# duylebkHCM/doc2tex

Hardware: AMD Instinct MI355X
Metric: formulas/s (greedy decode, 128x512 crops) (higher is better)
Workload: dtype bf16x3

## Files before the change

doc2tex_amd/csrc/decode.hip:

```cpp
#include <cstdlib>

#include "kernels.h"

namespace d2t {

using f32x4 = __attribute__((ext_vector_type(4))) float;
#ifndef D2T_DECODE_PRIO
#define D2T_DECODE_PRIO 3
#endif

__device__ __forceinline__ void decode_wave_priority() { __builtin_amdgcn_s_setprio(D2T_DECODE_PRIO); }

struct TraceScope {
  unsigned long long* t;
  __device__ __forceinline__ explicit TraceScope(unsigned long long* tr) : t(tr) {
    if (t && threadIdx.x == 0) atomicMin(t, (unsigned long long)__builtin_amdgcn_s_memrealtime());
  }
  __device__ __forceinline__ ~TraceScope() {
    if (t) {
      __syncthreads();
      if (threadIdx.x == 0) atomicMax(t + 1, (unsigned long long)__builtin_amdgcn_s_memrealtime());
    }
  }
};

__device__ __forceinline__ float act_fn(float v, int act) {
  if (act == ACT_RELU) return fmaxf(v, 0.f);
  if (act == ACT_GELU) return 0.5f * v * (1.f + erff(v * 0.70710678118654752440f));
  return v;
}

template <int NW, int NCH, int MT>
__global__ __launch_bounds__(NW * 64) void skinny_splitk_kernel(const SkinnyP p) {
  if (p.stop_at && *p.stop_at && *p.cur_step >= *p.stop_at) return;
  decode_wave_priority();
  TraceScope trace_(p.trace);
  constexpr int KS = NCH * 16;
  constexpr int ROWS = 16 * MT;
  __shared__ float part[NW][ROWS][17];
  __shared__ float stat[NW][ROWS];
  __shared__ float s_mean[ROWS], s_rstd[ROWS];
  const int tid = threadIdx.x, wave = tid >> 6, lane = tid & 63;
  const int r = lane & 15, q = lane >> 4;
  const int mbase = blockIdx.y * ROWS;
  const int n = blockIdx.x * 16 + r;
  const bool nok = n < p.N;
  const int k0 = wave * KS + q * 4;

  float4 a[MT][NCH], b[NCH];
#pragma unroll
  for (int i = 0; i < MT; ++i) {
    const int m = mbase + i * 16 + r;
    const bool mok = m < p.M;
    const float* src = p.x + (size_t)(mok ? m : 0) * p.ldx + k0;
#pragma unroll
    for (int c = 0; c < NCH; ++c) {
      a[i][c] = *reinterpret_cast<const float4*>(src + c * 16);
      if (!mok) a[i][c] = make_float4(0.f, 0.f, 0.f, 0.f);
    }
  }
  {
    const float* src = p.w + (size_t)(nok ? n : 0) * (p.wld ? p.wld : p.K) + k0;
#pragma unroll
    for (int c = 0; c < NCH; ++c) {
      b[c] = *reinterpret_cast<const float4*>(src + c * 16);
      if (!nok) b[c] = make_float4(0.f, 0.f, 0.f, 0.f);
    }
  }

  if (p.ln_g) {
    const float invK = 1.f / (float)p.K;
#pragma unroll
    for (int i = 0; i < MT; ++i) {
      float s = 0.f;
#pragma unroll
      for (int c = 0; c < NCH; ++c) s += (a[i][c].x + a[i][c].y) + (a[i][c].z + a[i][c].w);
      s += __shfl_xor(s, 16, 64);
      s += __shfl_xor(s, 32, 64);
      if (q == 0) stat[wave][i * 16 + r] = s;
    }
    __syncthreads();
    if (tid < ROWS) {
      float t = 0.f;
#pragma unroll
      for (int w = 0; w < NW; ++w) t += stat[w][tid];
      s_mean[tid] = t * invK;
    }
    __syncthreads();
#pragma unroll
    for (int i = 0; i < MT; ++i) {
      const float mu = s_mean[i * 16 + r];
      float s = 0.f;
#pragma unroll
      for (int c = 0; c < NCH; ++c) {
        a[i][c].x -= mu; a[i][c].y -= mu; a[i][c].z -= mu; a[i][c].w -= mu;
        s += (a[i][c].x * a[i][c].x + a[i][c].y * a[i][c].y) + (a[i][c].z * a[i][c].z + a[i][c].w * a[i][c].w);
      }
      s += __shfl_xor(s, 16, 64);
      s += __shfl_xor(s, 32, 64);
      if (q == 0) stat[wave][i * 16 + r] = s;
    }
    __syncthreads();
    if (tid < ROWS) {
      float t = 0.f;
#pragma unroll
      for (int w = 0; w < NW; ++w) t += stat[w][tid];
      s_rstd[tid] = 1.f / sqrtf(t * invK + p.ln_eps);
    }
    __syncthreads();
#pragma unroll
    for (int c = 0; c < NCH; ++c) {
      const float4 g4 = *reinterpret_cast<const float4*>(p.ln_g + k0 + c * 16);
      const float4 b4 = *reinterpret_cast<const float4*>(p.ln_b + k0 + c * 16);
#pragma unroll
      for (int i = 0; i < MT; ++i) {
        const float rs = s_rstd[i * 16 + r];
        a[i][c].x = a[i][c].x * rs * g4.x + b4.x;
        a[i][c].y = a[i][c].y * rs * g4.y + b4.y;
        a[i][c].z = a[i][c].z * rs * g4.z + b4.z;
        a[i][c].w = a[i][c].w * rs * g4.w + b4.w;
      }
    }
  }

  f32x4 acc[MT];
#pragma unroll
  for (int i = 0; i < MT; ++i) acc[i] = f32x4{0.f, 0.f, 0.f, 0.f};
#pragma unroll
  for (int c = 0; c < NCH; ++c) {
#pragma unroll
    for (int i = 0; i < MT; ++i) {
      acc[i] = __builtin_amdgcn_mfma_f32_16x16x4f32(a[i][c].x, b[c].x, acc[i], 0, 0, 0);
      acc[i] = __builtin_amdgcn_mfma_f32_16x16x4f32(a[i][c].y, b[c].y, acc[i], 0, 0, 0);
      acc[i] = __builtin_amdgcn_mfma_f32_16x16x4f32(a[i][c].z, b[c].z, acc[i], 0, 0, 0);
      acc[i] = __builtin_amdgcn_mfma_f32_16x16x4f32(a[i][c].w, b[c].w, acc[i], 0, 0, 0);
    }
  }
#pragma unroll
  for (int i = 0; i < MT; ++i)
#pragma unroll
    for (int reg = 0; reg < 4; ++reg) part[wave][i * 16 + q * 4 + reg][r] = acc[i][reg];
  __syncthreads();

  float* y = p.y;
  if (p.step_ptr) y += (long long)(*p.step_ptr) * p.out_step_stride;
  for (int idx = tid; idx < ROWS * 16; idx += NW * 64) {
    const int row = idx >> 4, col = idx & 15;
    const int m = mbase + row, nn = blockIdx.x * 16 + col;
    if (m >= p.M || nn >= p.N) continue;
    float v = 0.f;
#pragma unroll
    for (int w = 0; w < NW; ++w) v += part[w][row][col];
    v += p.bias ? p.bias[nn] : 0.f;
    if (p.res) v += p.res[(size_t)m * p.ldres + nn];
    y[(size_t)m * p.ldy + nn] = act_fn(v, p.act);
    if (p.ln_out && nn < p.K) {
      const float xv = p.x[(size_t)m * p.ldx + nn];
      p.ln_out[(size_t)m * p.K + nn] = (xv - s_mean[row]) * s_rstd[row] * p.ln_g[nn] + p.ln_b[nn];
    }
  }
}

__global__ __launch_bounds__(256) void skinny_generic_kernel(const SkinnyP p) {
  const int wave = threadIdx.x >> 6, lane = threadIdx.x & 63;
  const int r = lane & 15, q = lane >> 4;
  const int m = blockIdx.y * 64 + wave * 16 + r;
  const int n = blockIdx.x * 16 + r;
  const bool mok = m < p.M, nok = n < p.N;
  const float* xa = p.x + (size_t)(mok ? m : 0) * p.ldx + q * 4;
  const float* wb = p.w + (size_t)(nok ? n : 0) * p.K + q * 4;
  f32x4 acc = {0.f, 0.f, 0.f, 0.f};
  const int KC = p.K >> 4;
  for (int c = 0; c < KC; ++c) {
    float4 a = *reinterpret_cast<const float4*>(xa + c * 16);
    float4 b = *reinterpret_cast<const float4*>(wb + c * 16);
    if (!mok) a = make_float4(0.f, 0.f, 0.f, 0.f);
    if (!nok) b = make_float4(0.f, 0.f, 0.f, 0.f);
    acc = __builtin_amdgcn_mfma_f32_16x16x4f32(a.x, b.x, acc, 0, 0, 0);
    acc = __builtin_amdgcn_mfma_f32_16x16x4f32(a.y, b.y, acc, 0, 0, 0);
    acc = __builtin_amdgcn_mfma_f32_16x16x4f32(a.z, b.z, acc, 0, 0, 0);
    acc = __builtin_amdgcn_mfma_f32_16x16x4f32(a.w, b.w, acc, 0, 0, 0);
  }
  const int nn = blockIdx.x * 16 + r;
  if (nn >= p.N) return;
  float* y = p.y;
  if (p.step_ptr) y += (long long)(*p.step_ptr) * p.out_step_stride;
  const float bias = p.bias ? p.bias[nn] : 0.f;
#pragma unroll
  for (int reg = 0; reg < 4; ++reg) {
    const int mm = blockIdx.y * 64 + wave * 16 + q * 4 + reg;
    if (mm >= p.M) continue;
    float v = acc[reg] + bias;
    if (p.res) v += p.res[(size_t)mm * p.ldres + nn];
    y[(size_t)mm * p.ldy + nn] = act_fn(v, p.act);
  }
}

static int decode_small() {
  static const int v = D2T_PROBE_ENV("D2T_DECODE_SMALL");
  return v;
}

hipError_t launch_skinny(const SkinnyP& p, hipStream_t s) {
  if (p.M <= 0 || p.N <= 0) return hipSuccess;
  if (p.K % 16 != 0 || p.ldx % 4 != 0) return hipErrorInvalidValue;
  if (p.ln_out && (!p.ln_g || p.N < p.K)) return hipErrorInvalidValue;
  const int mt = p.N <= 512 ? 1 : 2;
  const dim3 grid((p.N + 15) / 16, (p.M + 16 * mt - 1) / (16 * mt));
#define D2T_SK(NW, NCH)                                                                                  \
  do {                                                                                                   \
    if (mt == 1) hipLaunchKernelGGL((skinny_splitk_kernel<NW, NCH, 1>), grid, dim3(NW * 64), 0, s, p);   \
    else hipLaunchKernelGGL((skinny_splitk_kernel<NW, NCH, 2>), grid, dim3(NW * 64), 0, s, p);           \
  } while (0)
  if (p.K == 256) D2T_SK(4, 4);
  else if (p.K == 512) D2T_SK(8, 4);
  else if (p.K == 1024 && decode_small() && !p.ln_g && !p.step_ptr) {
    SkinnyP a = p, b = p;
    a.K = 512; a.ldx = p.ldx; a.w = p.w; a.wld = p.K;
    b.K = 512; b.x = p.x + 512; b.w = p.w + 512; b.wld = p.K; b.bias = nullptr; b.res = p.y; b.ldres = p.ldy;
    a.act = ACT_NONE;
    if (p.act != ACT_NONE) return hipErrorInvalidValue;
    hipLaunchKernelGGL((skinny_splitk_kernel<4, 8, 1>), dim3((p.N + 15) / 16, (p.M + 15) / 16), dim3(256), 0, s, a);
    hipLaunchKernelGGL((skinny_splitk_kernel<4, 8, 1>), dim3((p.N + 15) / 16, (p.M + 15) / 16), dim3(256), 0, s, b);
  }
  else if (p.K == 1024) D2T_SK(8, 8);
  else {
    if (p.ln_g) return hipErrorInvalidValue;
    hipLaunchKernelGGL(skinny_generic_kernel, dim3((p.N + 15) / 16, (p.M + 63) / 64), dim3(256), 0, s, p);
  }
#undef D2T_SK
  return hipGetLastError();
}

template <int HD>
__global__ __launch_bounds__(256) void decode_attention_kernel(const DecAttnP p) {
  constexpr int LPK = HD / 4;
  constexpr int KPI = 64 / LPK;
  constexpr int MAXIT = 512 / (KPI * 4);
  __shared__ float w_m[4], w_s[4];
  __shared__ __attribute__((aligned(16))) float w_acc[4][HD];
  const int tid = threadIdx.x, wave = tid >> 6, lane = tid & 63;
  const int kig = lane / LPK, ch = lane % LPK;
  const int b = blockIdx.x / p.heads, head = blockIdx.x % p.heads;
  int L = p.L, t = -1;
  if (p.step_ptr) { t = *p.step_ptr; L = t + 1; }
  float* Kc = p.k + (size_t)b * p.kv_batch_stride + (size_t)head * p.Lmax * HD;
  float* Vc = p.v + (size_t)b * p.kv_batch_stride + (size_t)head * p.Lmax * HD;
  const float* curk = p.cur_k ? p.cur_k + (size_t)b * p.cur_stride + head * HD : nullptr;
  const float* curv = p.cur_v ? p.cur_v + (size_t)b * p.cur_stride + head * HD : nullptr;
  if (curk && t >= 0 && tid < HD) {
    Kc[(size_t)t * HD + tid] = curk[tid];
    Vc[(size_t)t * HD + tid] = curv[tid];
  }
  const float4 q4 = *reinterpret_cast<const float4*>(p.q + (size_t)b * p.q_stride + head * HD + ch * 4);
  const float scale = HD == 32 ? 0.17677669529663687f : 0.125f;
  const int nit = (L + KPI * 4 - 1) / (KPI * 4);

  float sc[MAXIT];
  float mloc = -INFINITY;
#pragma unroll
  for (int it = 0; it < MAXIT; ++it) {
    sc[it] = -INFINITY;
    if (it < nit) {
      const int j = (it * 4 + wave) * KPI + kig;
      float d = 0.f;
      if (j < L) {
        const float* kr = (curk && j == t) ? curk : Kc + (size_t)j * HD;
        const float4 k4 = *reinterpret_cast<const float4*>(kr + ch * 4);
        d = (q4.x * k4.x + q4.y * k4.y) + (q4.z * k4.z + q4.w * k4.w);
      }
#pragma unroll
      for (int o = 1; o < LPK; o <<= 1) d += __shfl_xor(d, o, 64);
      if (j < L) {
        sc[it] = d * scale;
        mloc = fmaxf(mloc, sc[it]);
      }
    }
  }
#pragma unroll
  for (int o = LPK; o < 64; o <<= 1) mloc = fmaxf(mloc, __shfl_xor(mloc, o, 64));
  float4 acc = make_float4(0.f, 0.f, 0.f, 0.f);
  float ssum = 0.f;
#pragma unroll
  for (int it = 0; it < MAXIT; ++it) {
    if (it < nit) {
      const int j = (it * 4 + wave) * KPI + kig;
      if (j < L) {
        const float pj = expf(sc[it] - mloc);
        const float* vr = (curv && j == t) ? curv : Vc + (size_t)j * HD;
        const float4 v4 = *reinterpret_cast<const float4*>(vr + ch * 4);
        ssum += pj;
        acc.x = fmaf(pj, v4.x, acc.x); acc.y = fmaf(pj, v4.y, acc.y);
        acc.z = fmaf(pj, v4.z, acc.z); acc.w = fmaf(pj, v4.w, acc.w);
      }
    }
  }
#pragma unroll
  for (int o = LPK; o < 64; o <<= 1) {
    ssum += __shfl_xor(ssum, o, 64);
    acc.x += __shfl_xor(acc.x, o, 64); acc.y += __shfl_xor(acc.y, o, 64);
    acc.z += __shfl_xor(acc.z, o, 64); acc.w += __shfl_xor(acc.w, o, 64);
  }
  if (kig == 0) *reinterpret_cast<float4*>(&w_acc[wave][ch * 4]) = acc;
  if (lane == 0) { w_m[wave] = mloc; w_s[wave] = ssum; }
  __syncthreads();
  if (tid < HD) {
    const float m = fmaxf(fmaxf(w_m[0], w_m[1]), fmaxf(w_m[2], w_m[3]));
    float tot = 0.f, o = 0.f;
#pragma unroll
    for (int w = 0; w < 4; ++w) {
      const float f = w_s[w] > 0.f ? expf(w_m[w] - m) : 0.f;
      tot += w_s[w] * f;
      o += w_acc[w][tid] * f;
    }
    p.y[(size_t)b * p.y_stride + head * HD + tid] = o / tot;
  }
}

hipError_t launch_decode_attention(const DecAttnP& p, hipStream_t s) {
  const int Lcap = p.step_ptr ? p.Lmax : p.L;
  if (Lcap > 512 || Lcap < 1) return hipErrorInvalidValue;
  const dim3 grid(p.B * p.heads);
  if (p.hd == 32) hipLaunchKernelGGL(decode_attention_kernel<32>, grid, dim3(256), 0, s, p);
  else if (p.hd == 64) hipLaunchKernelGGL(decode_attention_kernel<64>, grid, dim3(256), 0, s, p);
  else return hipErrorInvalidValue;
  return hipGetLastError();
}

__global__ void embed_kernel(const float* __restrict__ emb, const float* __restrict__ pe,
                             const int64_t* __restrict__ start, const int64_t* __restrict__ tokens, int tok_stride,
                             const int* __restrict__ step_ptr, float* __restrict__ x, int d, float sqrt_d) {
  const int b = blockIdx.x, t = *step_ptr;
  const int64_t tok = t == 0 ? start[b] : tokens[(size_t)b * tok_stride + t - 1];
  for (int c = threadIdx.x; c < d; c += blockDim.x)
    x[(size_t)b * d + c] = emb[(size_t)tok * d + c] * sqrt_d + pe[(size_t)t * d + c];
}

hipError_t launch_embed(const float* emb, const float* pe, const int64_t* start, const int64_t* tokens,
                        int tok_stride, const int* step_ptr, float* x, int B, int d, hipStream_t s) {
  hipLaunchKernelGGL(embed_kernel, dim3(B), dim3(256), 0, s, emb, pe, start, tokens, tok_stride, step_ptr, x, d,
                     sqrtf((float)d));
  return hipGetLastError();
}

__global__ __launch_bounds__(64) void argmax_embed_kernel(const ArgmaxP p) {
  const int t = *p.step_ptr;
  if (p.stop_at && *p.stop_at && t >= *p.stop_at) return;
  decode_wave_priority();
  TraceScope trace_(p.trace);
  const int b = blockIdx.x, lane = threadIdx.x;
  const float* row = p.logits + (size_t)b * p.row_stride + (size_t)t * p.step_stride;
  float best = -INFINITY;
  int bi = 0x7fffffff;
  for (int i = lane; i < p.V; i += 64) {
    const float v = row[i];
    if (v > best || (v == best && i < bi)) { best = v; bi = i; }
  }
#pragma unroll
  for (int o = 32; o > 0; o >>= 1) {
    const float ov = __shfl_xor(best, o, 64);
    const int oi = __shfl_xor(bi, o, 64);
    if (ov > best || (ov == best && oi < bi)) { best = ov; bi = oi; }
  }
  if (bi >= p.V) bi = 0;
  if (p.x) {
    const float sqrt_d = sqrtf((float)p.d);
    const float* e = p.emb + (size_t)bi * p.d;
    const float* pe = p.pe + (size_t)(t + 1) * p.d;
    for (int c = lane; c < p.d; c += 64) p.x[(size_t)b * p.d + c] = e[c] * sqrt_d + pe[c];
  }
  if (lane == 0) {
    p.tokens[(size_t)b * p.tok_stride + t] = bi;
    if (bi == p.end_token && !p.ended[b]) {
      p.ended[b] = 1;
      const int c = atomicAdd(p.end_count, 1) + 1;
      if (c == p.B) *p.steps_done = t + 1;
      if (p.n_batches > 0) {
        const int k = p.row_batch ? p.row_batch[b] : b / p.rows_per_batch;
        const int rows_k = p.batch_rows ? p.batch_rows[k] : p.rows_per_batch;
        const int nb = p.n_batches_ptr ? *p.n_batches_ptr : p.n_batches;
        if (atomicAdd(p.batch_end_count + k, 1) + 1 == rows_k) {
          p.batch_steps_done[k] = t + 1;
          if (atomicAdd(p.batches_done, 1) + 1 == nb && p.stop_at) *p.stop_at = t + 1;
        }
      }
    }
    __threadfence();
    if (atomicAdd(p.done_count, 1) == p.B - 1) {
      *p.done_count = 0;
      *p.step_ptr = t + 1;
    }
  }
}

hipError_t launch_argmax_embed(const ArgmaxP& p, hipStream_t s) {
  hipLaunchKernelGGL(argmax_embed_kernel, dim3(p.B), dim3(64), 0, s, p);
  return hipGetLastError();
}

__global__ __launch_bounds__(256) void ragged_finalize_kernel(int64_t* __restrict__ tokens, float* __restrict__ logits,
                                                              const int* __restrict__ row_batch, const int* __restrict__ batch_steps_done,
                                                              int S, int V) {
  const int b = blockIdx.x;
  const int n = batch_steps_done[row_batch[b]];
  if (n <= 0 || n >= S) return;
  for (int t = n + threadIdx.x; t < S; t += 256) tokens[(size_t)b * S + t] = 0;
  float* l = logits + ((size_t)b * S + n) * V;
  const size_t cnt = (size_t)(S - n) * V;
  for (size_t i = threadIdx.x; i < cnt; i += 256) l[i] = 0.f;
}

hipError_t launch_ragged_finalize(int64_t* tokens, float* logits, const int* row_batch, const int* batch_steps_done, int B, int S,
                                  int V, hipStream_t s) {
  if (B < 1) return hipSuccess;
  hipLaunchKernelGGL(ragged_finalize_kernel, dim3(B), dim3(256), 0, s, tokens, logits, row_batch, batch_steps_done, S, V);
  return hipGetLastError();
}

__device__ __forceinline__ float att_dot4(const float4& q, const float4& k) {
  return fmaf(q.x, k.x, q.y * k.y) + fmaf(q.z, k.z, q.w * k.w);
}
__device__ __forceinline__ void att_update(float sj, const float4& v, float& m, float& l, float4& acc) {
  const float mn = fmaxf(m, sj);
  const float f = expf(m - mn);
  const float pj = expf(sj - mn);
  l = fmaf(l, f, pj);
  acc.x = fmaf(pj, v.x, acc.x * f); acc.y = fmaf(pj, v.y, acc.y * f);
  acc.z = fmaf(pj, v.z, acc.z * f); acc.w = fmaf(pj, v.w, acc.w * f);
  m = mn;
}
__device__ __forceinline__ void att_merge(int o, float& m, float& l, float4& acc) {
  const float mo = __shfl_xor(m, o, 64), lo = __shfl_xor(l, o, 64);
  const float ax = __shfl_xor(acc.x, o, 64), ay = __shfl_xor(acc.y, o, 64);
  const float az = __shfl_xor(acc.z, o, 64), aw = __shfl_xor(acc.w, o, 64);
  const float mn = fmaxf(m, mo);
  const float f1 = l > 0.f ? expf(m - mn) : 0.f, f2 = lo > 0.f ? expf(mo - mn) : 0.f;
  l = fmaf(lo, f2, l * f1);
  acc.x = fmaf(ax, f2, acc.x * f1); acc.y = fmaf(ay, f2, acc.y * f1);
  acc.z = fmaf(az, f2, acc.z * f1); acc.w = fmaf(aw, f2, acc.w * f1);
  m = mn;
}

template <int HD, int U>
__device__ __forceinline__ void row_attention(const float* q, const float* Kc, const float* Vc, const float* curk,
                                              const float* curv, int t, int L, float* out, int lane,
                                              const int* anc = nullptr, long long anc_stride = 0) {
  constexpr int LPK = HD / 4, KPI = 64 / LPK;
  const int kig = lane / LPK, ch = lane % LPK;
  const float4 q4 = *reinterpret_cast<const float4*>(q + ch * 4);
  const float scale = HD == 32 ? 0.17677669529663687f : 0.125f;
  float m = -INFINITY, l = 0.f;
  float4 acc = make_float4(0.f, 0.f, 0.f, 0.f);
  const int nit = (L + KPI - 1) / KPI;
  for (int it0 = 0; it0 < nit; it0 += U) {
    float4 k4[U], v4[U];
#pragma unroll
    for (int u = 0; u < U; ++u) {
      const int j = (it0 + u) * KPI + kig;
      const int jj = j < L ? j : 0;
      const size_t ro = (anc && jj != t) ? (size_t)anc[jj] * (size_t)anc_stride : 0;
      const float* kr = (curk && jj == t) ? curk : Kc + ro + (size_t)jj * HD;
      const float* vr = (curv && jj == t) ? curv : Vc + ro + (size_t)jj * HD;
      k4[u] = *reinterpret_cast<const float4*>(kr + ch * 4);
      v4[u] = *reinterpret_cast<const float4*>(vr + ch * 4);
    }
#pragma unroll
    for (int u = 0; u < U; ++u) {
      const int j = (it0 + u) * KPI + kig;
      float d = HD == 64 ? att_dot4(q4, k4[u]) : (q4.x * k4[u].x + q4.y * k4[u].y) + (q4.z * k4[u].z + q4.w * k4[u].w);
#pragma unroll
      for (int o = 1; o < LPK; o <<= 1) d += __shfl_xor(d, o, 64);
      if (j < L) {
        if constexpr (HD == 64) {
          att_update(d * scale, v4[u], m, l, acc);
        } else {
          const float sj = d * scale;
          const float mn = fmaxf(m, sj);
          const float f = expf(m - mn);
          const float pj = expf(sj - mn);
          l = l * f + pj;
          acc.x = acc.x * f + pj * v4[u].x; acc.y = acc.y * f + pj * v4[u].y;
          acc.z = acc.z * f + pj * v4[u].z; acc.w = acc.w * f + pj * v4[u].w;
          m = mn;
        }
      }
    }
  }
#pragma unroll
  for (int o = LPK; o < 64; o <<= 1) {
    if constexpr (HD == 64) {
      att_merge(o, m, l, acc);
    } else {
      const float mo = __shfl_xor(m, o, 64), lo = __shfl_xor(l, o, 64);
      const float ax = __shfl_xor(acc.x, o, 64), ay = __shfl_xor(acc.y, o, 64);
      const float az = __shfl_xor(acc.z, o, 64), aw = __shfl_xor(acc.w, o, 64);
      const float mn = fmaxf(m, mo);
      const float f1 = l > 0.f ? expf(m - mn) : 0.f, f2 = lo > 0.f ? expf(mo - mn) : 0.f;
      l = l * f1 + lo * f2;
      acc.x = acc.x * f1 + ax * f2; acc.y = acc.y * f1 + ay * f2;
      acc.z = acc.z * f1 + az * f2; acc.w = acc.w * f1 + aw * f2;
      m = mn;
    }
  }
  if (kig == 0) {
    const float inv = 1.f / l;
    *reinterpret_cast<float4*>(out + ch * 4) = make_float4(acc.x * inv, acc.y * inv, acc.z * inv, acc.w * inv);
  }
}

#define ROW_KERNEL_ENTRY(p, dead_row)                                       \
  if ((p).stop_at && *(p).stop_at && *(p).step_ptr >= *(p).stop_at) return; \
  if (dead_row) return;                                                     \
  decode_wave_priority();                                                   \
  TraceScope trace_((p).trace)

__device__ __forceinline__ void fma4(float a, const float4& w, float4& acc) {
  acc.x = fmaf(a, w.x, acc.x); acc.y = fmaf(a, w.y, acc.y); acc.z = fmaf(a, w.z, acc.z); acc.w = fmaf(a, w.w, acc.w);
}
__device__ __forceinline__ float4 scale4(const float4& a, float s) { return make_float4(a.x * s, a.y * s, a.z * s, a.w * s); }

template <int D, int NTH, int CTX_HD = 0>
__device__ __forceinline__ void row_gemv(const float* in_s, const float* __restrict__ Wt, float* part_s, int tid) {
  constexpr int LPR = D / 4, G = NTH / LPR, KG = D / G;
  const int lr = tid % LPR, g = tid / LPR;
  const float* w = Wt + (size_t)(g * KG) * D + lr * 4;
  const float* in = in_s + (CTX_HD ? ((lr * 4) / CTX_HD) * D : 0) + g * KG;
  float4 acc = make_float4(0.f, 0.f, 0.f, 0.f);
#pragma unroll
  for (int k = 0; k < KG; ++k) fma4(in[k], *reinterpret_cast<const float4*>(w + (size_t)k * D), acc);
  *reinterpret_cast<float4*>(part_s + g * D + lr * 4) = acc;
}
template <int D, int NTH, int UNROLL>
__device__ __forceinline__ void gemv2(const float* in0, const float* in1, const float* __restrict__ Wt, float* part0, float* part1,
                                      int tid) {
  constexpr int LPR = D / 4, G = NTH / LPR, KG = D / G;
  const int lr = tid % LPR, g = tid / LPR;
  const float* w = Wt + (size_t)(g * KG) * D + lr * 4;
  float4 a0 = make_float4(0.f, 0.f, 0.f, 0.f), a1 = a0;
#pragma unroll UNROLL
  for (int k = 0; k < KG; ++k) {
    const float4 w4 = *reinterpret_cast<const float4*>(w + (size_t)k * D);
    const float x0 = in0[g * KG + k], x1 = in1[g * KG + k];
    fma4(x0, w4, a0);
    fma4(x1, w4, a1);
  }
  *reinterpret_cast<float4*>(part0 + g * D + lr * 4) = a0;
  *reinterpret_cast<float4*>(part1 + g * D + lr * 4) = a1;
}

template <int G, int D>
__device__ __forceinline__ float sum_parts(const float* part, int c, float v) {
#pragma unroll
  for (int g = 0; g < G; ++g) v += part[g * D + c];
  return v;
}

template <int D, class Gamma, class Beta>
__device__ __forceinline__ void row_ln1(const float* y_row, float* x1_row, int lane, float eps, Gamma gamma, Beta beta) {
  constexpr int V = D / 64;
  float v[V], s = 0.f;
#pragma unroll
  for (int i = 0; i < V; ++i) { v[i] = y_row[i * 64 + lane]; s += v[i]; }
#pragma unroll
  for (int o = 32; o > 0; o >>= 1) s += __shfl_xor(s, o, 64);
  const float mean = s * (1.f / D);
  float q = 0.f;
#pragma unroll
  for (int i = 0; i < V; ++i) { v[i] -= mean; q += v[i] * v[i]; }
#pragma unroll
  for (int o = 32; o > 0; o >>= 1) q += __shfl_xor(q, o, 64);
  const float rstd = 1.f / sqrtf(q * (1.f / D) + eps);
#pragma unroll
  for (int i = 0; i < V; ++i) {
    const int c = i * 64 + lane;
    x1_row[c] = v[i] * rstd * gamma(i, c) + beta(i, c);
  }
}
template <int D>
__device__ __forceinline__ void row_ln1(const float* y_row, float* x1_row, int lane, const DecRowP& p) {
  row_ln1<D>(y_row, x1_row, lane, p.eps, [&](int, int c) { return p.ln1_g[c]; }, [&](int, int c) { return p.ln1_b[c]; });
}

struct HeadPtrs { const float *q, *K, *V, *curk, *curv; };
template <int D, int HD>
__device__ __forceinline__ HeadPtrs cache_append_and_heads(const DecRowP& p, int b, int head, int t, int lane, bool store) {
  const float* qkv = p.qkv + (size_t)b * p.qkv_stride;
  float* Kc = p.sk + (size_t)b * p.s_batch_stride + (size_t)head * p.s_Lmax * HD;
  float* Vc = p.sv + (size_t)b * p.s_batch_stride + (size_t)head * p.s_Lmax * HD;
  const float* curk = qkv + D + head * HD;
  const float* curv = qkv + 2 * D + head * HD;
  if (lane < HD && store) {
    Kc[(size_t)t * HD + lane] = curk[lane];
    Vc[(size_t)t * HD + lane] = curv[lane];
  }
  return {qkv + head * HD, Kc, Vc, curk, curv};
}
struct HeadPair {
  const float *q[2], *K[2], *V[2], *curk[2], *curv[2];
  float* out[2];
  __device__ __forceinline__ void set(int i, const HeadPtrs& h, float* o) {
    q[i] = h.q; K[i] = h.K; V[i] = h.V; curk[i] = h.curk; curv[i] = h.curv; out[i] = o;
  }
};
template <int D, int HD, bool ANC = false>
__device__ __forceinline__ void row_self_attention(const DecRowP& p, int b, int head, int t, int lane, float* out,
                                                   const int* anc_s = nullptr) {
  const HeadPtrs h = cache_append_and_heads<D, HD>(p, b, head, t, lane, true);
  if (ANC && p.anc)
    row_attention<HD, 4>(h.q, p.sk + (size_t)head * p.s_Lmax * HD, p.sv + (size_t)head * p.s_Lmax * HD, h.curk, h.curv, t, t + 1, out,
                         lane, anc_s, p.s_batch_stride);
  else
    row_attention<HD, 4>(h.q, h.K, h.V, h.curk, h.curv, t, t + 1, out, lane);
}

template <int D, int HD, int NTH>
__global__ __launch_bounds__(NTH, NTH == 256 ? 4 : 2) void decoder_row_kernel(const DecRowP p) {
  constexpr int G = NTH / (D / 4);
  constexpr int HPW = 8 * 64 / NTH;
  ROW_KERNEL_ENTRY(p, false);
  __shared__ __attribute__((aligned(16))) float a_s[D], y_s[D], x1_s[D], q2_s[D], part_s[G * D];
  const int tid = threadIdx.x, wave = tid >> 6, lane = tid & 63;
  const int b = blockIdx.x;
  const int t = *p.step_ptr;
#pragma unroll
  for (int hp = 0; hp < HPW; ++hp) {
    const int head = wave + hp * (NTH / 64);
    row_self_attention<D, HD>(p, b, head, t, lane, a_s + head * HD);
  }
  __syncthreads();
  row_gemv<D, NTH>(a_s, p.wo_t, part_s, tid);
  __syncthreads();
  if (tid < D) y_s[tid] = sum_parts<G, D>(part_s, tid, p.bo[tid] + p.xres[(size_t)b * D + tid]);
  __syncthreads();
  if (wave == 0) row_ln1<D>(y_s, x1_s, lane, p);
  __syncthreads();
  row_gemv<D, NTH>(x1_s, p.wq_t, part_s, tid);
  __syncthreads();
  if (tid < D) q2_s[tid] = sum_parts<G, D>(part_s, tid, p.bq[tid]);
  __syncthreads();
#pragma unroll
  for (int hp = 0; hp < HPW; ++hp) {
    const int head = wave + hp * (NTH / 64);
    const int cb = p.c_row_map ? p.c_row_map[b] : b;
    const float* Kc = p.ck + (size_t)cb * p.c_batch_stride + (size_t)head * p.T * HD;
    const float* Vc = p.cv + (size_t)cb * p.c_batch_stride + (size_t)head * p.T * HD;
    row_attention<HD, 8>(q2_s + head * HD, Kc, Vc, nullptr, nullptr, -1, p.T, a_s + head * HD, lane);
  }
  __syncthreads();
  row_gemv<D, NTH>(a_s, p.wco_t, part_s, tid);
  __syncthreads();
  if (tid < D) p.y2[(size_t)b * D + tid] = sum_parts<G, D>(part_s, tid, p.bco[tid] + x1_s[tid]);
}

typedef __attribute__((address_space(3))) void* lds_ptr_dec;

#ifdef D2T_PROBES
__device__ unsigned long long d2t_row_phase[32];
#define ROW_PHASE(k) do { if (blockIdx.x == 0 && threadIdx.x == 0) { const unsigned long long now_ = __builtin_amdgcn_s_memrealtime(); \
    atomicAdd(&d2t_row_phase[k], now_ - phase_t_); phase_t_ = now_; } } while (0)
#define ROW_PHASE_INIT() unsigned long long phase_t_ = __builtin_amdgcn_s_memrealtime(); if (blockIdx.x == 0 && threadIdx.x == 0) atomicAdd(&d2t_row_phase[31], 1ull)
#define WAVE_PHASE(k) do { if (blockIdx.x == 0 && threadIdx.x == 0) { const unsigned long long now_ = __builtin_amdgcn_s_memrealtime(); \
    atomicAdd(&d2t_row_phase[k], now_ - wave_t_); wave_t_ = now_; } } while (0)
#define WAVE_PHASE_INIT() unsigned long long wave_t_ = __builtin_amdgcn_s_memrealtime()
#define ROW_PROBE(bit) (p.probe & (bit))
#else
#define ROW_PHASE(k) do { } while (0)
#define ROW_PHASE_INIT() do { } while (0)
#define WAVE_PHASE(k) do { } while (0)
#define WAVE_PHASE_INIT() do { } while (0)
#define ROW_PROBE(bit) 0
#endif

// ... 1154 lines not shown
```

Measured before the change: 1629.

## Hoist global loads ahead of stop check and sync in decode kernels

The skinny split-K GEMM gets an LN template parameter. All global loads (activations, weights, LN gamma/beta, bias, residual, LN side inputs, stop flags) are issued before the early-exit check and the barriers, and the LN mean and rstd are reduced redundantly per lane, which removes two __syncthreads per LN pass. The argmax+embed kernel likewise batches logits and positional-encoding loads into unrolled register arrays when V and d are small. The aim is to hide memory latency in these latency-bound decode kernels, at the cost of higher register pressure, loads that are wasted when a block exits early, and explicit occupancy hints.

Result: no change. 1641 (median of 6 runs) (+0.7%).

```diff
diff --git a/doc2tex_amd/csrc/decode.hip b/doc2tex_amd/csrc/decode.hip
--- a/doc2tex_amd/csrc/decode.hip
+++ b/doc2tex_amd/csrc/decode.hip
@@ -30,15 +30,21 @@
   return v;
 }
 
-template <int NW, int NCH, int MT>
-__global__ __launch_bounds__(NW * 64) void skinny_splitk_kernel(const SkinnyP p) {
-  if (p.stop_at && *p.stop_at && *p.cur_step >= *p.stop_at) return;
+__device__ __forceinline__ float sq4_sum(const float4& v) {
+#pragma clang fp contract(off)
+  return (v.x * v.x + v.y * v.y) + (v.z * v.z + v.w * v.w);
+}
+
+template <int NW, int NCH, int MT, bool LN>
+__global__ __launch_bounds__(NW * 64, (LN && NCH == 8) ? 1 : (NCH == 8 && MT == 2) ? 3 : 4)
+void skinny_splitk_kernel(const SkinnyP p) {
   decode_wave_priority();
-  TraceScope trace_(p.trace);
+  constexpr bool LN_EARLY = LN && NCH <= 4, EPI_EARLY = !LN || NCH <= 4;
   constexpr int KS = NCH * 16;
   constexpr int ROWS = 16 * MT;
+  constexpr int EPT = (ROWS * 16 + NW * 64 - 1) / (NW * 64);
   __shared__ float part[NW][ROWS][17];
-  __shared__ float stat[NW][ROWS];
+  __shared__ __attribute__((aligned(16))) float stat[2][ROWS][NW];
   __shared__ float s_mean[ROWS], s_rstd[ROWS];
   const int tid = threadIdx.x, wave = tid >> 6, lane = tid & 63;
   const int r = lane & 15, q = lane >> 4;
@@ -47,29 +53,73 @@
   const bool nok = n < p.N;
   const int k0 = wave * KS + q * 4;
 
-  float4 a[MT][NCH], b[NCH];
+  const int* const dummy = reinterpret_cast<const int*>(p.w);
+  const bool stoppable = p.stop_at && p.cur_step;
+  const int stop_v = *(stoppable ? p.stop_at : dummy), cur_v = *(stoppable ? p.cur_step : dummy);
+  const int step_v = *(p.step_ptr ? p.step_ptr : dummy);
+  float4 a[MT][NCH], b[NCH], g4[NCH], b4[NCH];
 #pragma unroll
   for (int i = 0; i < MT; ++i) {
     const int m = mbase + i * 16 + r;
-    const bool mok = m < p.M;
-    const float* src = p.x + (size_t)(mok ? m : 0) * p.ldx + k0;
+    const float* src = p.x + (size_t)(m < p.M ? m : 0) * p.ldx + k0;
+#pragma unroll
+    for (int c = 0; c < NCH; ++c) a[i][c] = *reinterpret_cast<const float4*>(src + c * 16);
+  }
+  if constexpr (LN_EARLY) {
 #pragma unroll
     for (int c = 0; c < NCH; ++c) {
-      a[i][c] = *reinterpret_cast<const float4*>(src + c * 16);
-      if (!mok) a[i][c] = make_float4(0.f, 0.f, 0.f, 0.f);
+      g4[c] = *reinterpret_cast<const float4*>(p.ln_g + k0 + c * 16);
+      b4[c] = *reinterpret_cast<const float4*>(p.ln_b + k0 + c * 16);
     }
   }
   {
     const float* src = p.w + (size_t)(nok ? n : 0) * (p.wld ? p.wld : p.K) + k0;
 #pragma unroll
-    for (int c = 0; c < NCH; ++c) {
-      b[c] = *reinterpret_cast<const float4*>(src + c * 16);
-      if (!nok) b[c] = make_float4(0.f, 0.f, 0.f, 0.f);
-    }
-  }
-
-  if (p.ln_g) {
+    for (int c = 0; c < NCH; ++c) b[c] = *reinterpret_cast<const float4*>(src + c * 16);
+  }
+  const int e_nn0 = blockIdx.x * 16;
+  float e_bias[EPT], e_res[EPT], e_x[EPT], e_g[EPT], e_b[EPT];
+  const bool ln_side = LN && p.ln_out != nullptr;
+#pragma unroll
+  for (int e = 0; e < EPT; ++e) {
+    const int idx = tid + e * NW * 64;
+    const int m = mbase + (idx >> 4), nn = e_nn0 + (idx & 15);
+    const bool ok = idx < ROWS * 16 && m < p.M && nn < p.N;
+    const int mc = ok ? m : mbase, nc = ok ? nn : e_nn0;
+    e_bias[e] = 0.f; e_res[e] = 0.f; e_x[e] = 0.f; e_g[e] = 0.f; e_b[e] = 0.f;
+    if constexpr (EPI_EARLY) {
+      e_bias[e] = *(p.bias ? p.bias + nc : p.w);
+      e_res[e] = *(p.res ? p.res + (size_t)mc * p.ldres + nc : p.w);
+      if constexpr (LN) {
+        const int kc = nc < p.K ? nc : 0;
+        e_x[e] = p.x[(size_t)mc * p.ldx + kc];
+        e_g[e] = p.ln_g[kc];
+        e_b[e] = p.ln_b[kc];
+      }
+    }
+  }
+
+  asm volatile("" ::: "memory");
+  if (stoppable && stop_v && cur_v >= stop_v) return;
+  TraceScope trace_(p.trace);
+#pragma unroll
+  for (int i = 0; i < MT; ++i)
+    if (mbase + i * 16 + r >= p.M) {
+#pragma unroll
+      for (int c = 0; c < NCH; ++c) a[i][c] = make_float4(0.f, 0.f, 0.f, 0.f);
+    }
+
+  if constexpr (LN) {
     const float invK = 1.f / (float)p.K;
+    auto row_total = [&](int pass, int row) {
+      float t = 0.f;
+#pragma unroll
+      for (int w4 = 0; w4 < NW; w4 += 4) {
+        const float4 v = *reinterpret_cast<const float4*>(&stat[pass][row][w4]);
+        t += v.x; t += v.y; t += v.z; t += v.w;
+      }
+      return t;
+    };
 #pragma unroll
     for (int i = 0; i < MT; ++i) {
       float s = 0.f;
@@ -77,50 +127,49 @@
       for (int c = 0; c < NCH; ++c) s += (a[i][c].x + a[i][c].y) + (a[i][c].z + a[i][c].w);
       s += __shfl_xor(s, 16, 64);
       s += __shfl_xor(s, 32, 64);
-      if (q == 0) stat[wave][i * 16 + r] = s;
+      if (q == 0) stat[0][i * 16 + r][wave] = s;
     }
     __syncthreads();
-    if (tid < ROWS) {
-      float t = 0.f;
-#pragma unroll
-      for (int w = 0; w < NW; ++w) t += stat[w][tid];
-      s_mean[tid] = t * invK;
-    }
-    __syncthreads();
+    float mu[MT], rs[MT];
 #pragma unroll
     for (int i = 0; i < MT; ++i) {
-      const float mu = s_mean[i * 16 + r];
+      mu[i] = row_total(0, i * 16 + r) * invK;
+      asm("" : "+v"(mu[i]));
       float s = 0.f;
 #pragma unroll
       for (int c = 0; c < NCH; ++c) {
-        a[i][c].x -= mu; a[i][c].y -= mu; a[i][c].z -= mu; a[i][c].w -= mu;
-        s += (a[i][c].x * a[i][c].x + a[i][c].y * a[i][c].y) + (a[i][c].z * a[i][c].z + a[i][c].w * a[i][c].w);
+        a[i][c].x -= mu[i]; a[i][c].y -= mu[i]; a[i][c].z -= mu[i]; a[i][c].w -= mu[i];
+        s += sq4_sum(a[i][c]);
       }
       s += __shfl_xor(s, 16, 64);
       s += __shfl_xor(s, 32, 64);
-      if (q == 0) stat[wave][i * 16 + r] = s;
+      if (q == 0) stat[1][i * 16 + r][wave] = s;
     }
     __syncthreads();
-    if (tid < ROWS) {
-      float t = 0.f;
-#pragma unroll
-      for (int w = 0; w < NW; ++w) t += stat[w][tid];
-      s_rstd[tid] = 1.f / sqrtf(t * invK + p.ln_eps);
-    }
-    __syncthreads();
+#pragma unroll
+    for (int i = 0; i < MT; ++i) {
+      rs[i] = 1.f / sqrtf(row_total(1, i * 16 + r) * invK + p.ln_eps);
+      asm("" : "+v"(rs[i]));
+      if (ln_side && wave == 0 && q == i) { s_mean[i * 16 + r] = mu[i]; s_rstd[i * 16 + r] = rs[i]; }
+    }
 #pragma unroll
     for (int c = 0; c < NCH; ++c) {
-      const float4 g4 = *reinterpret_cast<const float4*>(p.ln_g + k0 + c * 16);
-      const float4 b4 = *reinterpret_cast<const float4*>(p.ln_b + k0 + c * 16);
+      if constexpr (!LN_EARLY) {
+        g4[c] = *reinterpret_cast<const float4*>(p.ln_g + k0 + c * 16);
+        b4[c] = *reinterpret_cast<const float4*>(p.ln_b + k0 + c * 16);
+      }
 #pragma unroll
       for (int i = 0; i < MT; ++i) {
-        const float rs = s_rstd[i * 16 + r];
-        a[i][c].x = a[i][c].x * rs * g4.x + b4.x;
-        a[i][c].y = a[i][c].y * rs * g4.y + b4.y;
-        a[i][c].z = a[i][c].z * rs * g4.z + b4.z;
-        a[i][c].w = a[i][c].w * rs * g4.w + b4.w;
-      }
-    }
+        a[i][c].x = a[i][c].x * rs[i] * g4[c].x + b4[c].x;
+        a[i][c].y = a[i][c].y * rs[i] * g4[c].y + b4[c].y;
+        a[i][c].z = a[i][c].z * rs[i] * g4[c].z + b4[c].z;
+        a[i][c].w = a[i][c].w * rs[i] * g4[c].w + b4[c].w;
+      }
+    }
+  }
+  if (!nok) {
+#pragma unroll
+    for (int c = 0; c < NCH; ++c) b[c] = make_float4(0.f, 0.f, 0.f, 0.f);
   }
 
   f32x4 acc[MT];
@@ -143,21 +192,29 @@
   __syncthreads();
 
   float* y = p.y;
-  if (p.step_ptr) y += (long long)(*p.step_ptr) * p.out_step_stride;
-  for (int idx = tid; idx < ROWS * 16; idx += NW * 64) {
+  if (p.step_ptr) y += (long long)step_v * p.out_step_stride;
+#pragma unroll
+  for (int e = 0; e < EPT; ++e) {
+    const int idx = tid + e * NW * 64;
     const int row = idx >> 4, col = idx & 15;
-    const int m = mbase + row, nn = blockIdx.x * 16 + col;
-    if (m >= p.M || nn >= p.N) continue;
+    const int m = mbase + row, nn = e_nn0 + col;
+    if (idx >= ROWS * 16 || m >= p.M || nn >= p.N) continue;
     float v = 0.f;
 #pragma unroll
     for (int w = 0; w < NW; ++w) v += part[w][row][col];
-    v += p.bias ? p.bias[nn] : 0.f;
-    if (p.res) v += p.res[(size_t)m * p.ldres + nn];
+    if constexpr (!EPI_EARLY) {
+      if (p.bias) e_bias[e] = p.bias[nn];
+      if (p.res) e_res[e] = p.res[(size_t)m * p.ldres + nn];
+      if (ln_side && nn < p.K) {
+        e_x[e] = p.x[(size_t)m * p.ldx + nn];
+        e_g[e] = p.ln_g[nn];
+        e_b[e] = p.ln_b[nn];
+      }
+    }
+    v += p.bias ? e_bias[e] : 0.f;
+    if (p.res) v += e_res[e];
     y[(size_t)m * p.ldy + nn] = act_fn(v, p.act);
-    if (p.ln_out && nn < p.K) {
-      const float xv = p.x[(size_t)m * p.ldx + nn];
-      p.ln_out[(size_t)m * p.K + nn] = (xv - s_mean[row]) * s_rstd[row] * p.ln_g[nn] + p.ln_b[nn];
-    }
+    if (ln_side && nn < p.K) p.ln_out[(size_t)m * p.K + nn] = (e_x[e] - s_mean[row]) * s_rstd[row] * e_g[e] + e_b[e];
   }
 }
 
@@ -209,8 +266,10 @@
   const dim3 grid((p.N + 15) / 16, (p.M + 16 * mt - 1) / (16 * mt));
 #define D2T_SK(NW, NCH)                                                                                  \
   do {                                                                                                   \
-    if (mt == 1) hipLaunchKernelGGL((skinny_splitk_kernel<NW, NCH, 1>), grid, dim3(NW * 64), 0, s, p);   \
-    else hipLaunchKernelGGL((skinny_splitk_kernel<NW, NCH, 2>), grid, dim3(NW * 64), 0, s, p);           \
+    if (mt == 1 && p.ln_g) hipLaunchKernelGGL((skinny_splitk_kernel<NW, NCH, 1, true>), grid, dim3(NW * 64), 0, s, p);   \
+    else if (mt == 1) hipLaunchKernelGGL((skinny_splitk_kernel<NW, NCH, 1, false>), grid, dim3(NW * 64), 0, s, p);     \
+    else if (p.ln_g) hipLaunchKernelGGL((skinny_splitk_kernel<NW, NCH, 2, true>), grid, dim3(NW * 64), 0, s, p);       \
+    else hipLaunchKernelGGL((skinny_splitk_kernel<NW, NCH, 2, false>), grid, dim3(NW * 64), 0, s, p);                  \
   } while (0)
   if (p.K == 256) D2T_SK(4, 4);
   else if (p.K == 512) D2T_SK(8, 4);
@@ -220,8 +279,8 @@
     b.K = 512; b.x = p.x + 512; b.w = p.w + 512; b.wld = p.K; b.bias = nullptr; b.res = p.y; b.ldres = p.ldy;
     a.act = ACT_NONE;
     if (p.act != ACT_NONE) return hipErrorInvalidValue;
-    hipLaunchKernelGGL((skinny_splitk_kernel<4, 8, 1>), dim3((p.N + 15) / 16, (p.M + 15) / 16), dim3(256), 0, s, a);
-    hipLaunchKernelGGL((skinny_splitk_kernel<4, 8, 1>), dim3((p.N + 15) / 16, (p.M + 15) / 16), dim3(256), 0, s, b);
+    hipLaunchKernelGGL((skinny_splitk_kernel<4, 8, 1, false>), dim3((p.N + 15) / 16, (p.M + 15) / 16), dim3(256), 0, s, a);
+    hipLaunchKernelGGL((skinny_splitk_kernel<4, 8, 1, false>), dim3((p.N + 15) / 16, (p.M + 15) / 16), dim3(256), 0, s, b);
   }
   else if (p.K == 1024) D2T_SK(8, 8);
   else {
@@ -344,17 +403,45 @@
 }
 
 __global__ __launch_bounds__(64) void argmax_embed_kernel(const ArgmaxP p) {
+  const int stop = p.stop_at ? *p.stop_at : 0;
   const int t = *p.step_ptr;
-  if (p.stop_at && *p.stop_at && t >= *p.stop_at) return;
+  if (stop && t >= stop) return;
   decode_wave_priority();
   TraceScope trace_(p.trace);
   const int b = blockIdx.x, lane = threadIdx.x;
   const float* row = p.logits + (size_t)b * p.row_stride + (size_t)t * p.step_stride;
+  constexpr int U = 8;
+  const bool small_v = p.V <= U * 64, small_d = p.x && p.d <= U * 64;
+  float lv[U], pev[U];
+  if (small_v) {
+#pragma unroll
+    for (int j = 0; j < U; ++j) {
+      const int i = lane + j * 64;
+      lv[j] = row[i < p.V ? i : 0];
+    }
+  }
+  if (small_d) {
+    const float* pe = p.pe + (size_t)(t + 1) * p.d;
+#pragma unroll
+    for (int j = 0; j < U; ++j) {
+      const int c = lane + j * 64;
+      pev[j] = pe[c < p.d ? c : 0];
+    }
+  }
   float best = -INFINITY;
   int bi = 0x7fffffff;
-  for (int i = lane; i < p.V; i += 64) {
-    const float v = row[i];
-    if (v > best || (v == best && i < bi)) { best = v; bi = i; }
+  if (small_v) {
+#pragma unroll
+    for (int j = 0; j < U; ++j) {
+      const int i = lane + j * 64;
+      const float v = lv[j];
+      if (i < p.V && (v > best || (v == best && i < bi))) { best = v; bi = i; }
+    }
+  } else {
+    for (int i = lane; i < p.V; i += 64) {
+      const float v = row[i];
+      if (v > best || (v == best && i < bi)) { best = v; bi = i; }
+    }
   }
 #pragma unroll
   for (int o = 32; o > 0; o >>= 1) {
@@ -366,8 +453,22 @@
   if (p.x) {
     const float sqrt_d = sqrtf((float)p.d);
     const float* e = p.emb + (size_t)bi * p.d;
-    const float* pe = p.pe + (size_t)(t + 1) * p.d;
-    for (int c = lane; c < p.d; c += 64) p.x[(size_t)b * p.d + c] = e[c] * sqrt_d + pe[c];
+    if (small_d) {
+      float ev[U];
+#pragma unroll
+      for (int j = 0; j < U; ++j) {
+        const int c = lane + j * 64;
+        ev[j] = e[c < p.d ? c : 0];
+      }
+#pragma unroll
+      for (int j = 0; j < U; ++j) {
+        const int c = lane + j * 64;
+        if (c < p.d) p.x[(size_t)b * p.d + c] = ev[j] * sqrt_d + pev[j];
+      }
+    } else {
+      const float* pe = p.pe + (size_t)(t + 1) * p.d;
+      for (int c = lane; c < p.d; c += 64) p.x[(size_t)b * p.d + c] = e[c] * sqrt_d + pe[c];
+    }
   }
   if (lane == 0) {
     p.tokens[(size_t)b * p.tok_stride + t] = bi;
```
